# l646773422/h264-lab

Measured on AMD Instinct MI355X. Metric: 1080p macroblocks/sec, higher is better.
Workload: dtype u8

## Files before the change

h264-lab_amd/csrc/enc_mb.h:

```cpp
#ifndef H264E_ENC_MB_H
#define H264E_ENC_MB_H

#include <stddef.h>
#include "enc_kernels.h"

struct GCtx { mv32 mv_left[4], mv_tl[4], mv_top[8]; };
#define GSCR_OFF(t) ((t) == 0 ? 0 : (t) == 1 ? 1024 : (t) == 2 ? 1536 : 2048)
#define GSCR_BYTES 2304

struct MbBuf
{
    alignas(16) uint8_t inp[256];
    alignas(16) uint8_t inp_c[128];
    alignas(16) uint8_t pred[256];
    alignas(4) uint8_t pix_top[36];
    alignas(4) uint8_t ptop[96];
    mv32 mv_top[8];
    uint8_t nnz_top[8];
    int8_t i4_top[4];
    uint32_t df_nz_top;
    int top_type, top_qp;
    mv32 mv[16], mvd[16];
    int type, cost, used_cand;
    mv32 mv_skip_pred;
// ... 248 lines not shown
        v = mvadd(mv, mvmk(DX(pri) + DX(sec), DY(pri) + DY(sec)));
        if (in_rect(v, range))
        {
            cost = grp_sad_ref(R, px + (mvx(v) >> 2), py + (mvy(v) >> 2), b, w, h) + mv_cost(m, v, mv_pred);
            if (cost < min_sad)
            {
                mv = v;
                min_sad = cost;
                continue;
            }
        }
        break;
    }
    STAMP(L, 25);
#undef SEL4
#undef DX
#undef DY

#ifdef H264E_ABLATE
    if (H264E_ABLATE == 3) { grp_interp_luma(R, px, py, mv, w, h, dst); return min_sad; }
#endif
    if (!(m.speed < 9 && in_rect(mv, mv_qlimit(m))))
    {
        grp_interp_luma(R, px, py, mv, w, h, dst);
        return min_sad;
    }
    {
        mv32 pq = mvmk(0, -1), sq = mvmk(-1, 0);
        uint32_t ms1 = c1, ms2 = c3;
        if (c3 >= c2) { pq = mvmk(0, 1); ms2 = c2; }
        if (c1 >= c0) { sq = mvmk(1, 0); ms1 = c0; }
        if (ms2 > ms1) { mv32 sw = sq; sq = pq; pq = sw; }
        const mv32 vdg = mvadd(pq, sq);
        const mv32 v02 = mvadd(mv, mvadd(pq, pq)), v01 = mvadd(mv, pq), v20 = mvadd(mv, mvadd(sq, sq)), v10 = mvadd(mv, sq);
        const mv32 v11 = mvadd(mv, vdg), v22 = mvadd(mv, mvadd(vdg, vdg)), v12 = mvadd(mv, mvadd(pq, vdg));
        int s8[8];
        const int fx0 = px + (mvx(mv) >> 2), fy0 = py + (mvy(mv) >> 2), plane = w*h;
        const bool inside = rv_inside(R, fx0 - 5, fy0 - 3, fx0 + w + 4, fy0 + h + 3);
        if (!inside) rv_wait_rect_g(R, fy0 - 3, fx0 + w + 4, fy0 + h + 3);
        const int hp_ox = mvx(vdg) < 0 ? 1 : 0, hp_oy = mvy(vdg) < 0 ? 1 : 0, hp_pq_vertical = mvx(pq) == 0;
#define AVG4(x, y) (((x) | (y)) - ((((x) ^ (y)) >> 1) & 0x7f7f7f7fu))
        grp_sum8([&](int i, int *sv) {
            uint32_t t0 = 0, t1 = 0, t2 = 0, t3 = 0, t4 = 0, t5 = 0, t6 = 0;
            const int c4 = i & (g - 1), r0 = (i >> (g >> 1))*npass;
            const auto probe = [&](int r, uint32_t q00, uint32_t q02, uint32_t q20, uint32_t q22) {
                const int o = w*r + 4*c4;
                const uint32_t in4 = lds32(b + 16*r + 4*c4);
                const uint32_t q01 = AVG4(q00, q02), q10 = AVG4(q00, q20), q11 = AVG4(q02, q20), q12 = AVG4(q22, q02);
                lds32_store(scr + o, q00); lds32_store(scr + plane + o, q02); lds32_store(scr + 2*plane + o, q20); lds32_store(scr + 3*plane + o, q22);
                t0 = sad4_u8(q02, in4, t0); t1 = sad4_u8(q01, in4, t1); t2 = sad4_u8(q20, in4, t2);
                t3 = sad4_u8(q10, in4, t3); t4 = sad4_u8(q11, in4, t4); t5 = sad4_u8(q22, in4, t5);
                t6 = sad4_u8(q12, in4, t6);
            };
            if (inside)
            {
                halfpel3_rows(rv_ptr(R, fx0 + 4*c4 - hp_ox, fy0 + r0 - hp_oy), hp_ox, hp_oy, npass, [&](int k, const hp4_t &hp) {
                    probe(r0 + k, hp.x, hp_pq_vertical ? hp.z : hp.y, hp_pq_vertical ? hp.y : hp.z, hp.w);
                });
            } else
            {
                for (int k = 0; k < npass; k++)
                {
                    const int r = r0 + k;
#define IP(vv) interp_luma4(R, false, px + (mvx(vv) >> 2) + 4*c4, py + (mvy(vv) >> 2) + r, mvx(vv) & 3, mvy(vv) & 3)
                    const uint32_t q00 = IP(mv), q02 = IP(v02), q20 = IP(v20), q22 = IP(v22);
#undef IP
                    probe(r, q00, q02, q20, q22);
                }
            }
            sv[0] = (int)t0; sv[1] = (int)t1; sv[2] = (int)t2; sv[3] = (int)t3; sv[4] = (int)t4; sv[5] = (int)t5; sv[6] = (int)t6;
        }, s8);
        wave_sync();
        int best = -1, c8[8];
        mv32 vbest = mv;
        {
            const int pax = hp_pq_vertical, p_step = pax ? mvy(pq) : mvx(pq), s_step = pax ? mvx(sq) : mvy(sq);
            const int p_mv = pax ? mvy(mv) : mvx(mv), s_mv = pax ? mvx(mv) : mvy(mv), p_pr = pax ? mvy(mv_pred) : mvx(mv_pred), s_pr = pax ? mvx(mv_pred) : mvy(mv_pred);
            int P[4], S[4];
            grp_eval4([&](int k) -> int { return se_len((int16_t)(p_mv + k*p_step) - p_pr); }, P);
            grp_eval4([&](int k) -> int { return se_len((int16_t)(s_mv + k*s_step) - s_pr); }, S);
            c8[0] = MUL_LAMBDA(P[2] + S[0], m.lambda_mv); c8[1] = MUL_LAMBDA(P[1] + S[0], m.lambda_mv); c8[2] = MUL_LAMBDA(P[0] + S[2], m.lambda_mv);
            c8[3] = MUL_LAMBDA(P[0] + S[1], m.lambda_mv); c8[4] = MUL_LAMBDA(P[1] + S[1], m.lambda_mv); c8[5] = MUL_LAMBDA(P[2] + S[2], m.lambda_mv);
            c8[6] = MUL_LAMBDA(P[2] + S[1], m.lambda_mv);
        }
#define TRY(j, vv) { const int cst = s8[j] + c8[j]; if (cst < min_sad) { min_sad = cst; vbest = (vv); best = j; } }
        TRY(0, v02) TRY(1, v01) TRY(2, v20) TRY(3, v10) TRY(4, v11) TRY(5, v22) TRY(6, v12)
#undef TRY
        const int pa = best < 0 ? 0 : best == 0 ? 1 : best == 1 ? 0 : best == 2 ? 2 : best == 3 ? 0 : best == 4 ? 1 : best == 5 ? 3 : 3;
        const int pb = best == 1 ? 1 : best == 3 ? 2 : best == 4 ? 2 : best == 6 ? 1 : pa;
        GRP_FOR(i)
        {
            for (int k = 0; k < npass; k++)
            {
                const int d = i + 16*k, r = d >> (g >> 1), c4 = d & (g - 1), o = w*r + 4*c4;
                const uint32_t x = lds32(scr + pa*plane + o), y = lds32(scr + pb*plane + o);
                lds32_store(dst + 16*r + 4*c4, AVG4(x, y));
            }
        }
#undef AVG4
        wave_sync();
        mv = vbest;
    }
    STAMP(L, 26);
    return min_sad;
}

DEV void search_type(RowLds &L, const MbBuf &B, const MbCtx &m, int t, mv32 mv_best, int sad_best0, const rect_t &lim, int skip_cost)
{
    GCtx &X = L.gctx[t];
    int imv = 0, part_sad = MUL_LAMBDA(t == 0 ? 1 : t == 3 ? 12 : 4, m.lambda_q4);
    const int w = (t & 2) ? 8 : 16, h = (t & 1) ? 8 : 16;
    int px = 0, py = 0;
    uint8_t *test = L.gtest[t], *scr = L.gscr + GSCR_OFF(t);
    for (;;)
    {
        rect_t range;
        mv32 mvabs = mb_abs(m, mv_best);
        int sad_best = sad_best0;
        const mv32 mvp = mvp_get_arr(X.mv_left, X.mv_tl, X.mv_top, m.avail, px >> 2, py >> 2, w >> 2, h >> 2);
        if (!t) set_range(mvabs, range, lim, m.y*64 + py*4);
        else
        {
            mvabs = mvround(mb_abs(m, mvp));
            set_range(mvabs, range, lim, m.y*64 + py*4);
            sad_best = grp_sad_ref(m.rv, px + (mvx(mvabs) >> 2), py + (mvy(mvabs) >> 2), B.inp + 16*py + px, w, h)
                     + mv_cost(m, mvabs, mb_abs(m, mvp));
        }
        STAMP(L, 24);
        part_sad += diamond_g(L, B, m, px, py, mvabs, range, mb_abs(m, mvp), sad_best, w, h, test + 16*py + px, scr);
        const mv32 mv = mvsub(mvabs, mvmk(m.x*64, m.y*64));
        L.part_mvd[t][imv] = mvsub(mv, mvp);
        L.part_mv[t][imv++] = mv;
        mvp_put_arr(X.mv_left, X.mv_tl, X.mv_top, px >> 2, py >> 2, w >> 2, h >> 2, mv);
        wave_sync();
        STAMP(L, 27);
        if (t == 0) L.early_bound = imax(part_sad, skip_cost);
        px = (px + w) & 15;
        if (!px)
        {
            py = (py + h) & 15;
            if (!py) break;
        }
    }
    L.gcost[t] = part_sad;
    L.gnum[t] = imv;
}

DEV void partition_hints(const int sad[4], int mode[4])
{
    int sum = sad[0] + sad[1] + sad[2] + sad[3];
    int slope = iabs((sad[0] - sad[2]) + (sad[1] - sad[3])) - iabs((sad[0] - sad[1]) + (sad[2] - sad[3]));
    int skew = iabs(sad[3] - sad[0]) - iabs(sad[2] - sad[1]);
    if (slope > (sum >> 4)) mode[1] = 1;
    if (slope < -(sum >> 4)) mode[2] = 1;
    if (iabs(skew) > (sum >> 4) && iabs(slope) <= (sum >> 4)) mode[3] = 1;
}

DEV void predict_chroma_inter(const MbBuf &B, const MbCtx &m, uint8_t *pred_c)
{
    int w = (m.type & 2) ? 4 : 8, h = (m.type & 1) ? 4 : 8, part = 0, x = 0, y = 0;
    if (m.type == -1) w = h = 8;
    for (;; part++)
    {
        wave_interp_chroma(m.rv, m.ref[1], m.ref[2], x, y, mb_abs(m, B.mv[part]), w, h, pred_c + 16*y + x);
        x = (x + w) & 7;
        if (!x)
        {
            y = (y + h) & 7;
            if (!y) break;
        }
    }
}

DEV int skip_chroma_ok(const MbBuf &B, const MbCtx &m, const uint8_t *pred_c)
{
    const int thr = m.skip_thr;
    for (int c = 0; c < 2; c++)
    {
// ... 114 lines not shown
        if (kmin != 0x7fffffff && (kmin >> 4) < sad_best + cand_cost_best)
        {
            mv_best = (mv32)cand.get(kmin & 15);
            cand_cost_best = mv_cost(m, mv_best, mv_pred16);
            sad_best = (kmin >> 4) - cand_cost_best;
        }
    }
    sad_best += mv_cost(m, mv_best, mv_pred16);
    {
        int u = MUL_LAMBDA(1, m.lambda_q4) + sad_best;
        if (sad_skip != 0x7FFFFFFF) u = imax(u, sad_skip + mv_cost(m, mv_skip, mv_pred16));
        sig.bound(u);
    }
    STAMP(L, 4);

#ifdef H264E_ABLATE
    if (H264E_ABLATE == 1) prefer[3] = 0;
    if (H264E_ABLATE == 4) prefer[1] = prefer[2] = prefer[3] = 0;
#endif
    const int types = 1 | (prefer[1] ? 2 : 0) | (prefer[2] ? 4 : 0) | (prefer[3] ? 8 : 0);
#ifdef H264E_TYPES_PROBE
    PCOUNT(L, 20 + (types == 1 ? 0 : (types & 8) ? 2 : 1));
#endif
    WAVE_FOR(l)
    {
        const int i = l & 15;
        mv32 *c = &L.gctx[l >> 4].mv_left[0];
        c[i] = i < 4 ? L.mv_left[i] : i < 8 ? L.mv_tl[i - 4] : i < 13 ? B.mv_top[i - 8] : 0;
    }
    wave_sync();
    const bool helped = sig.helper() && (types & 8);
    if (helped) sig.t3_request(mv_best, sad_best, lim);
    const int types_here = helped ? types & 7 : types;
    GRP_EACH(t)
    {
        if ((types_here >> t) & 1) search_type(L, B, m, t, mv_best, sad_best, lim, sad_skip != 0x7FFFFFFF ? sad_skip + mv_cost(m, mv_skip, mv_pred16) : 0);
    }
    wave_sync();
    if (helped && !sig.t3_wait()) { m.type = 0; m.cost = 0xffffff; B.mv[0] = 0; B.mvd[0] = 0; return; }
    STAMP(L, 5);
    m.cost = 0xffffff;
    int best_n = 0;
    for (int t = 0; t < 4; t++)
        if ((types >> t) & 1)
        {
            const int c = uni(L.gcost[t]);
            if (c < m.cost) { m.cost = c; m.type = t; best_n = uni(L.gnum[t]); }
        }
    wave_copy_wh(B.pred, L.gtest[m.type], 16, 16);
    for (int i = 0; i < best_n; i++) { B.mv[i] = L.part_mv[m.type][i]; B.mvd[i] = L.part_mvd[m.type][i]; }
    wave_sync();

    if (m.cost > sad_skip)
    {
        m.type = 0;
        m.cost = sad_skip + mv_cost(m, mv_skip, mv_pred16);
        B.mv[0] = mv_skip;
        B.mvd[0] = mvsub(mv_skip, mv_pred16);
        wave_copy_wh(B.pred, L.skip_pred, 16, 16);
    }
}


DEV int intra16_cost(RowLds &L, const MbBuf &B, MbCtx &m)
{
    const uint8_t *p = B.inp;
    const int v = m.avail & 3;
    int mode, sad4[4];
    int dx = iabs(p[0] - p[15]) + iabs(p[15*16] - p[15*16 + 15]) + iabs(p[8*16] - p[8*16 + 15]);
// ... 322 lines not shown
```

h264-lab_amd/csrc/enc_row.h:

```cpp
#ifndef H264E_ENC_ROW_H
#define H264E_ENC_ROW_H

#include "enc_mb.h"

#define GEOM_WIDE 0
#define GEOM_NARROW 1
#define GEOM_INTRA 2

struct ChainG
{
    GLOBAL_AS h264e_mbbottom_t *bottom;
    GLOBAL_AS h264e_mbpend_t *pend;
    GLOBAL_AS int *progress;
    GLOBAL_AS uint32_t *rowbits;
    GLOBAL_AS h264e_rowmeta_t *rowmeta;
    GLOBAL_AS h264e_mbrec_t *mbrec;
    GLOBAL_AS uint8_t *arena;
    uint32_t arena_cap;
    GLOBAL_AS uint8_t *nal_arena;
    uint32_t nal_cap;
    GLOBAL_AS uint32_t *cursor;
    GLOBAL_AS h264e_frameout_t *fout;
    GLOBAL_AS int *far_reads;
    unsigned long long *prof;
};
DEV ChainG chain_view(const h264e_chain_dev_t &C)
{
    ChainG g;
    g.bottom = (GLOBAL_AS h264e_mbbottom_t *)C.bottom; g.pend = (GLOBAL_AS h264e_mbpend_t *)C.pend; g.progress = (GLOBAL_AS int *)C.progress;
    g.rowbits = (GLOBAL_AS uint32_t *)C.rowbits; g.rowmeta = (GLOBAL_AS h264e_rowmeta_t *)C.rowmeta;
    g.mbrec = (GLOBAL_AS h264e_mbrec_t *)C.mbrec; g.arena = (GLOBAL_AS uint8_t *)C.arena; g.arena_cap = C.arena_cap; g.nal_arena = (GLOBAL_AS uint8_t *)C.nal_arena; g.nal_cap = C.nal_cap;
    g.cursor = (GLOBAL_AS uint32_t *)C.cursor; g.fout = (GLOBAL_AS h264e_frameout_t *)C.fout; g.far_reads = (GLOBAL_AS int *)C.far_reads; g.prof = C.prof;
    return g;
}

DEV void row_begin(RowLds &L, const h264e_geom_t &G, const ChainG &C, const h264e_frame_task_t &T, int row)
{
    WAVE_FOR(l)
    {
        if (l < 4) { L.mv_left[l] = 0; L.mv_tl[l] = 0; L.i4_left[l] = -1; L.pix_tl[l] = 0; }
        if (l < 8) L.nnz_left[l] = NNZ_NA;
        if (l < 32) L.pix_left[l] = 0;
        if (l < 25) L.df_mv[l] = 0;
        L.strip_y[l] = 0;
        L.strip_c[l >> 5][l & 31] = 0;
    }
    L.df_nzflag = 0;
    L.left_type = 0;
    L.left_qp = T.qp;
    L.bw.acc = 0; L.bw.nacc = 0; L.bw.pos = 0; L.bw.overflow = 0;
    L.bw.cap = (uint32_t)G.row_words;
    L.bw.buf = C.rowbits + (size_t)row*G.row_words;
    L.skip_run = 0; L.lead_skips = 0; L.coded_any = 0; L.far_reads[0] = L.far_reads[1] = L.far_reads[2] = 0; L.far_fail[0] = L.far_fail[1] = L.far_fail[2] = 0;
    L.f_noskip = L.f_bound = L.f_inter = L.f_decided = L.f_wdone = L.f_stop = 0; L.early_bound = 0; L.f_t3req = L.f_t3done = L.f_front = 0;
    WAVE_FOR(l) { if (l <= H264E_MAX_SLICES) L.slice_row[l] = l <= T.nslices ? T.slice_row[l] : (int16_t)0x7fff; }
    WAVE_FOR(l)
    {
        for (int k = l; k < 84; k += 64) L.qdat[k/42][k%42] = T.qdat[k/42][k%42];
    }
    cavlc_tab_load(L.cavlc);
    df_tab_load(L.dftab);
    L.qconst[0] = k_lambda_mv_q4[T.qp]; L.qconst[1] = k_lambda_q4[T.qp]; L.qconst[2] = k_skip_thr_inter[T.qp];
    L.qconst[3] = k_skip_thr_i4x4[T.qp]; L.qconst[4] = k_lambda_i4_q4[T.qp]; L.qconst[5] = k_lambda_i16_q4[T.qp];
    L.win_x = -2;
#ifdef H264E_STAMPS
// ... 734 lines not shown
```

h264-lab_amd/csrc/h264e_kernels.hip:

```cpp
#include <stdio.h>
#include <stdlib.h>
#include <string.h>
#include "enc_row.h"
#include "enc_selftest.h"
#include "enc_denoise.h"
#include "enc_ingest.h"
#include "enc_egress.h"
#include "enc_scale.h"
#include "enc_scale_rgb.h"
#include "enc_hbd.h"
#include "enc_scenecut.h"
#include "enc_ssim.h"
#include "../../include/h264e_hip.h"

#include <hip/hip_runtime.h>





#ifndef H264E_POLL_SLEEP
#define H264E_POLL_SLEEP 16
#endif
DEV int poll_progress(const GLOBAL_AS int *flag, int need, int &seen, unsigned spin_limit)
// ... 46 lines not shown
};
struct InterFromSearchWave
{
    RowLds *L;
    int need;
    bool back_wave;
    DEVM bool before_decide() const { return !back_wave || need < 2 || lds_wait(&L->f_wdone, need - 1, &L->f_stop) == 0; }
    DEVM bool ready() const { return uni(flag_get(&L->f_inter)) >= need; }
    DEVM bool wait_ready() const { return lds_wait(&L->f_inter, need, &L->f_stop) == 0; }
    DEVM int early_bound() const { return uni(flag_get(&L->f_bound)) >= need ? uni(L->early_bound) : 0x7fffffff; }
    DEVM bool wait_either(const int *f) const
    {
        for (unsigned spins = 0;; spins++)
        {
            if (uni(flag_get(&L->f_inter)) >= need || uni(flag_get(f)) >= need) return true;
            if (uni(flag_get(&L->f_stop))) return false;
            if (spins > LDS_SPIN_LIMIT) { flag_set(&L->f_stop, -1); return false; }
            __builtin_amdgcn_s_sleep(H264E_LDS_SLEEP);
        }
    }
    DEVM bool wait_noskip_or_ready() const { return wait_either(&L->f_noskip); }
    DEVM bool wait_bound_or_ready() const { return wait_either(&L->f_bound); }
};

#ifndef H264E_WPE2
#define H264E_WPE2 3
#endif
#ifndef H264E_WPE1
#define H264E_WPE1 2
#endif
#ifndef H264E_WPEI
#define H264E_WPEI 4
#endif
template <int GEOM, int WAVES, int OCC>
__global__ void __launch_bounds__(64*WAVES, OCC) h264e_mb_kernel(h264e_geom_t G, const h264e_frame_task_t *tasks, const uint32_t *order)
{
    __shared__ __attribute__((aligned(16))) unsigned char L_bytes[GEOM == GEOM_INTRA ? ROWLDS_INTRA_BYTES : sizeof(RowLds)];
    RowLds &L = *reinterpret_cast<RowLds *>(L_bytes);
    const int wv = WAVES >= 2 ? __builtin_amdgcn_readfirstlane((int)(threadIdx.x >> 6)) : 0;
#ifdef H264E_LDS_PAD
    __shared__ volatile char lds_pad[H264E_LDS_PAD];
    if (G.nmbx < 0) lds_pad[LANE] = 1;
#endif
    const uint32_t jr = order[blockIdx.x];
    if (jr == H264E_ORDER_PAD) return;
    const int job = (int)(jr >> 16), row = (int)(jr & 0xffffu);
    const h264e_frame_task_t &T = tasks[job];
    if (!T.active) return;
    const ChainG C = chain_view(*T.chain_desc);
    GLOBAL_AS int *errflag = (GLOBAL_AS int *)uniptr(T.errflag);

    if (row == G.nmby)
    {
        if (wv) return;
#ifdef H264E_STAMPS
        unsigned long long fz_t = wall_clock64();
#define FZ_STAMP(id) do { const unsigned long long n_ = wall_clock64(); if (LANE == 0 && C.prof) atomicAdd(C.prof + (id), n_ - fz_t); fz_t = n_; } while (0)
#else
#define FZ_STAMP(id) do { } while (0)
#endif
        int st = 0, seen = 0;
        GLOBAL_AS h264e_hostdone_t *hd = (GLOBAL_AS h264e_hostdone_t *)T.host_done;
        GLOBAL_AS h264e_walkrec_t *wout = (GLOBAL_AS h264e_walkrec_t *)T.walk_out;
        int wstatus = 0, first_bad = -1, have_prev = !(T.walk_on_device && T.walk_prev), published = 0;
        mv32 ws[2] = { T.exact_state[0], T.exact_state[1] };
        const GLOBAL_AS h264e_walkrec_t *wp = (const GLOBAL_AS h264e_walkrec_t *)T.walk_prev;
        const GLOBAL_AS h264e_mbrec_t *rec = C.mbrec + (size_t)T.frame_slot*G.nmb;
        JobWalk W;
        W.begin(ws);
        const bool state_fixed = T.nslices > 1;
        const auto take_prev = [&]() {
            __builtin_amdgcn_fence(__ATOMIC_ACQUIRE, "agent");
            asm volatile("s_waitcnt vmcnt(0)" ::: "memory");
            __builtin_amdgcn_wave_barrier();
            if (uni(wp->status) != H264E_WALK_OK) wstatus = H264E_WALK_VOID;
            else if (!state_fixed) { ws[0] = (mv32)uni(wp->state_out[0]); ws[1] = (mv32)uni(wp->state_out[1]); W.begin(ws); }
            have_prev = 1;
// ... 136 lines not shown
    if (row < T.first_row) return;
    if (job == 0 && row == G.test_stall_row) return;
    if (wv == 0) row_begin(L, G, C, T, row);
    if (WAVES >= 2) __syncthreads();
    const RowTask RT = rowtask_load(T);
    int row0 = 0, row1 = G.nmby;
    for (int k = 0; k < T.nslices; k++)
        if (row >= T.slice_row[k] && row < T.slice_row[k + 1]) { row0 = T.slice_row[k]; row1 = T.slice_row[k + 1]; }
    row0 = uni(row0); row1 = uni(row1);
    GLOBAL_AS int *my_progress = C.progress + row;
    GLOBAL_AS unsigned long long *mb_counter = (GLOBAL_AS unsigned long long *)uniptr(T.mb_counter);
    const auto count_mbs = [&](int n) { if (mb_counter && n > 0 && LANE == 0) __hip_atomic_fetch_add(mb_counter, (unsigned long long)n, __ATOMIC_RELAXED, __HIP_MEMORY_SCOPE_AGENT); };

    if (WAVES == 1 || wv == 0)
    {
        const GLOBAL_AS int *abort_word = (const GLOBAL_AS int *)uniptr(T.abort_word);
        const int launch_id = uni(T.launch_id);
        int seen = 0, seen_dep = 0;
        constexpr bool NARROW = GEOM == GEOM_NARROW;
        constexpr int DEP_ROWS = NARROW ? H264E_NARROW_DEP_ROWS : H264E_DEP_ROWS, DEP_COLS = NARROW ? H264E_NARROW_DEP_COLS : H264E_DEP_COLS;
        unsigned long long deps = 0;
        int ndeps = 0;
        if (T.dep_progress)
        {
            const int lo = imax(row - 2, 0), hi = imin(row + DEP_ROWS, G.nmby - 1);
            deps = (unsigned long long)hi; ndeps = 1;
            for (int k = T.nslices - 1; k >= 1; k--)
            {
                const int last = T.slice_row[k] - 1;
                if (last >= lo && last < hi) { deps |= (unsigned long long)last << (10*ndeps); ndeps++; }
            }
            ndeps = uni(ndeps);
        }
        for (int x = 0; x < G.nmbx; x++)
        {
            const int need = row > row0 ? imin(x + 2, G.nmbx) : 0;
            const int need_dep = RT.dep_progress ? imin(x + DEP_COLS, G.nmbx) : 0;
            int st = 0;
            const int abort_v = abort_word ? __hip_atomic_load(abort_word, __ATOMIC_RELAXED, __HIP_MEMORY_SCOPE_AGENT) : launch_id - 1;
            const GLOBAL_AS int *above = C.progress + (WAVES >= 2 ? G.nmby : 0) + (row - 1);
            const int early = seen < need ? __hip_atomic_load(above, __ATOMIC_RELAXED, __HIP_MEMORY_SCOPE_AGENT) : seen;
            if (seen_dep < need_dep)
            {
                int lowest = 0x7fffffff;
                for (int k = 0; k < ndeps && !st; k++)
                {
                    int sk = 0;
                    st = poll_progress((const GLOBAL_AS int *)RT.dep_progress + (int)((deps >> (10*k)) & 1023), need_dep, sk, G.spin_limit);
                    lowest = imin(lowest, sk);
                }
                seen_dep = lowest;
                if (!st) consumer_acquire();
            }
            STAMP(L, 13);
            if (WAVES >= 2 && !st && x >= 2) st = lds_wait(&L.f_wdone, x - 1, &L.f_stop);
            STAMP(L, 23);
            if (!st) row_prefetch<GEOM>(L, G, RT, row, x);
            STAMP(L, 0);
            if (uni(abort_v) == launch_id) st = -2;
            if (!st && seen < need)
            {
                seen = uni(early);
                if (seen < 0) st = seen;
                else if (seen < need) st = poll_progress(above, need, seen, G.spin_limit);
                if (!st) consumer_acquire();
            }
            STAMP(L, 13);
            if (!st) load_top<WAVES >= 2 ? LOAD_TOP_MV : LOAD_TOP_ALL>(L, L.mb[x & 1], G, C.bottom + (size_t)(row - 1)*G.nmbx, C.pend + (size_t)(row - 1)*G.nmbx, x, row > row0);
            STAMP(L, 0);
            if (WAVES >= 2 && !st && x >= 1) st = lds_wait(&L.f_decided, x, &L.f_stop);
            STAMP(L, 6);
            if (st)
            {
                if (WAVES >= 2) { flag_set(&L.f_stop, st); return; }
                if (LANE == 0)
                {
                    if (st == -1) *errflag = 1;
                    __hip_atomic_store(my_progress, st, __ATOMIC_RELAXED, __HIP_MEMORY_SCOPE_AGENT);
                }
                count_mbs(x);
                return;
            }
            if (WAVES == 1) row_step<GEOM>(L, G, C, RT, row, x, row0, row1);
            else mb_search<GEOM>(L, L.mb[x & 1], G, RT, row, x, row0, SearchSignals{ &L, x + 1, WAVES >= 3 });
            if (WAVES >= 3 && uni(flag_get(&L.f_stop))) return;
            {
                const int ff = uni(L.far_fail[0]) | (WAVES == 1 ? uni(L.far_fail[1]) : 0);
                if (ff)
                {
                    if (WAVES >= 2) { flag_set(&L.f_stop, ff < -2 ? -2 : ff); return; }
                    if (LANE == 0)
                    {
                        if (ff == -1) *errflag = 1;
                        __hip_atomic_store(my_progress, ff < -2 ? -2 : ff, __ATOMIC_RELAXED, __HIP_MEMORY_SCOPE_AGENT);
                    }
                    count_mbs(x);
                    return;
                }
            }
            if (WAVES >= 2) { flag_set(&L.f_inter, x + 1); STAMP(L, 14); continue; }
            asm volatile("s_waitcnt vmcnt(0)" ::: "memory");
// ... 459 lines not shown
```

h264-lab_amd/csrc/h264e_pool.h:

```cpp
#ifndef H264E_POOL_H
#define H264E_POOL_H
#include "enc_denoise.h"
#include "enc_ingest.h"
#include "enc_egress.h"
#include "enc_scale.h"
#include "enc_scale_rgb.h"
#include "enc_hbd.h"
#include "enc_scenecut.h"
#include "enc_ssim.h"

static const h264e_color_t k_color_rows[4] = {
    { { 66, 129, 25 }, { -38, -74, 112 }, { 112, -94, -18 }, 16 },
    { { 77, 150, 29 }, { -43, -84, 127 }, { 127, -107, -20 }, 0 },
    { { 47, 157, 16 }, { -26, -86, 112 }, { 112, -102, -10 }, 16 },
    { { 54, 183, 19 }, { -29, -98, 127 }, { 127, -116, -11 }, 0 } };

static const h264e_icolor_t k_icolor_rows[4] = {
    { 298, 16, 409, -100, -208, 516 },
    { 256, 0, 359, -88, -183, 454 },
    { 298, 16, 459, -55, -136, 541 },
    { 256, 0, 403, -48, -120, 475 } };

static thread_local char g_err[256];
#define FAIL(...) do { snprintf(g_err, sizeof(g_err), __VA_ARGS__); return -1; } while (0)
// ... 1294 lines not shown
        (void)hipMemset(p->errflag, 0, sizeof(int));
        FAIL("macroblock kernel gave up waiting for the row above (bounded spin expired)");
    }
    device_release(p);
    p->pending = 0;
    return 0;
}

extern "C" void h264e_hip_release(h264e_hip_pool_t *p)
{
    if (!p) return;
    (void)hipSetDevice(p->device);
    if (p->stream) (void)hipStreamSynchronize(p->stream);
    device_release(p);
}


extern "C" int h264e_hip_group_create(h264e_hip_group_t **out, int device)
{
    if (!out) FAIL("group_create: null argument");
    h264e_hip_group_t *g = (h264e_hip_group_t *)calloc(1, sizeof(*g));
    if (!g) FAIL("out of host memory");
    g->device = device;
    pthread_mutex_init(&g->mu, 0); pthread_cond_init(&g->cv, 0);
    if (hipSetDevice(device) != hipSuccess || hipStreamCreate(&g->stream) != hipSuccess) { free(g); FAIL("group_create: no stream on device %d", device); }
    (void)hipEventCreate(&g->ev_done);
    for (int k = 0; k < 2; k++) { (void)hipEventCreate(&g->ev_t0[k]); (void)hipEventCreate(&g->ev_t1[k]); }
    *out = g;
    return 0;
}

#define H264E_RESIDENT_WG_V2 1536
#define H264E_RESIDENT_WG_V3 512
static int pick_variant(const launch_shape_t &s, int jobs, int nmby)
{
    if (s.forced) return s.forced;
    if (s.all_intra) return 0;
    if (jobs*nmby >= H264E_RESIDENT_WG_V2 && s.parallel && !s.tree) return 4;
    if (jobs*(nmby + 1) <= H264E_RESIDENT_WG_V3) return 3;
    return 2;
}

static hipError_t launch_mb(const h264e_geom_t &G, int narrow, int variant, int jobs, size_t nblocks, const h264e_frame_task_t *tasks, const uint32_t *order,
                            hipEvent_t before, hipEvent_t after, hipStream_t stream)
{
    hipError_t e = before ? hipEventRecord(before, stream) : hipSuccess;
    if (e != hipSuccess) return e;
    bk_launch_mb(G, narrow, variant, jobs, (unsigned)nblocks, tasks, order, stream);
    e = after ? hipEventRecord(after, stream) : hipSuccess;
    const hipError_t le = hipGetLastError();
    return le != hipSuccess ? le : e;
}

static int group_fail(h264e_hip_group_t *g, const char *fmt, ...)
{
    va_list ap;
    va_start(ap, fmt);
    vsnprintf(g->err, sizeof(g->err), fmt, ap);
    va_end(ap);
    return -1;
}

static int group_grow(h264e_hip_group_t *g, void **buf, size_t *cap, size_t need, size_t slack, size_t elem)
{
    if (need <= *cap) return 0;
    if (*buf) (void)hipFree(*buf);
    *cap = need + slack;
    if (hipMalloc(buf, elem**cap) == hipSuccess) return 0;
    *buf = 0; *cap = 0;
    return group_fail(g, "group launch: device allocation failed");
}
// ... 556 lines not shown
```

h264-lab_amd/csrc/wave.h:

```cpp
#ifndef H264E_WAVE_H
#define H264E_WAVE_H

#include <stdint.h>
#include <string.h>

#ifdef H264E_EMU
extern "C" void emu_check_global(const void *p, size_t n, const char *file, int line);
#define EMU_GLOBAL(p, n) emu_check_global((const void *)(p), (n), __FILE__, __LINE__)
#define GLOBAL_AS
#define LDS_AS
#define NOINLINE_DEV static __attribute__((noinline))
#define DEV static inline
#define DEVM inline
#define DCONST static const
#ifdef H264E_EMU_REVERSE
#define WAVE_FOR(l) for (int l = 63; l >= 0; --l)
#else
#define WAVE_FOR(l) for (int l = 0; l < 64; ++l)
#endif
struct u32x4 { uint32_t x, y, z, w; };
DEV void wave_sync() {}
DEV int wave_lane() { return 0; }
DEV int uni(int v) { return v; }
template <class F> DEV int wave_sum(F f)
// ... 11 lines not shown
        f(l, v);
        for (int k = 0; k < 4; ++k) out[k] += v[k];
    }
}
template <class F> DEV void wave_sum8(F f, int out[8])
{
    for (int k = 0; k < 8; ++k) out[k] = 0;
    for (int l = 0; l < 64; ++l)
    {
        int v[8] = { 0, 0, 0, 0, 0, 0, 0, 0 };
        f(l, v);
        for (int k = 0; k < 8; ++k) out[k] += v[k];
    }
}
template <class F> DEV uint64_t wave_ballot(F f)
{
    uint64_t m = 0;
    for (int l = 0; l < 64; ++l) if (f(l)) m |= 1ull << l;
    return m;
}
DEV uint32_t sad4_u8(uint32_t a, uint32_t b, uint32_t acc)
{
    for (int k = 0; k < 4; ++k)
    {
        int d = (int)((a >> (8*k)) & 255) - (int)((b >> (8*k)) & 255);
        acc += (uint32_t)(d < 0 ? -d : d);
    }
    return acc;
}
DEV int clz32(uint32_t v) { return __builtin_clz(v); }
DEV uint32_t bswap32(uint32_t v) { return __builtin_bswap32(v); }

#define GRP_EACH(g) for (int g = 0; g < 4; ++g)
#ifdef H264E_EMU_REVERSE
#define GRP_FOR(i) for (int i = 15; i >= 0; --i)
#else
#define GRP_FOR(i) for (int i = 0; i < 16; ++i)
#endif
template <class F> DEV int grp_sum(F f)
{
    int s = 0;
    for (int i = 0; i < 16; ++i) s += f(i);
    return s;
}
template <class F> DEV void grp_sum4(F f, int out[4])
{
    out[0] = out[1] = out[2] = out[3] = 0;
    for (int i = 0; i < 16; ++i)
    {
        int v[4] = { 0, 0, 0, 0 };
        f(i, v);
        for (int k = 0; k < 4; ++k) out[k] += v[k];
    }
}
template <class F> DEV void grp_sum8(F f, int out[8])
{
    for (int k = 0; k < 8; ++k) out[k] = 0;
    for (int i = 0; i < 16; ++i)
    {
        int v[8] = { 0, 0, 0, 0, 0, 0, 0, 0 };
        f(i, v);
        for (int k = 0; k < 8; ++k) out[k] += v[k];
    }
}
template <class F> DEV void grp_eval4(F f, int out[4]) { for (int d = 0; d < 4; ++d) out[d] = f(d); }
template <class F> DEV void grp_eval8(F f, int out[8]) { for (int d = 0; d < 8; ++d) out[d] = f(d); }
DEV void grp_count(int *p) { *p += 1; }

struct V16 { int v[16]; };
#define V16_BINOP(op) DEV V16 operator op(const V16 &a, const V16 &b) { V16 r; for (int i = 0; i < 16; i++) r.v[i] = a.v[i] op b.v[i]; return r; }
V16_BINOP(+) V16_BINOP(-) V16_BINOP(*) V16_BINOP(&) V16_BINOP(|)
#undef V16_BINOP
DEV V16 operator>>(const V16 &a, int s) { V16 r; for (int i = 0; i < 16; i++) r.v[i] = a.v[i] >> s; return r; }
DEV V16 v16_splat(int s) { V16 r; for (int i = 0; i < 16; i++) r.v[i] = s; return r; }
template <class F> DEV V16 v16_make(F f) { V16 r; for (int i = 0; i < 16; i++) r.v[i] = f(i, 0); return r; }
template <class F> DEV V16 v16_map(const V16 &a, F f) { V16 r; for (int i = 0; i < 16; i++) r.v[i] = f(i, a.v[i]); return r; }
template <class F> DEV V16 v16_map2(const V16 &a, const V16 &b, F f) { V16 r; for (int i = 0; i < 16; i++) r.v[i] = f(i, a.v[i], b.v[i]); return r; }
template <class F> DEV V16 v16_map3(const V16 &a, const V16 &b, const V16 &c, F f) { V16 r; for (int i = 0; i < 16; i++) r.v[i] = f(i, a.v[i], b.v[i], c.v[i]); return r; }
template <class F> DEV void v16_each(const V16 &a, F f) { for (int i = 0; i < 16; i++) f(i, 0, a.v[i]); }
DEV int v16_any(const V16 &a) { for (int i = 0; i < 16; i++) if (a.v[i]) return 1; return 0; }
DEV V16 v16_tile_any(const V16 &a) { V16 r; const int n = v16_any(a); for (int i = 0; i < 16; i++) r.v[i] = n; return r; }
DEV unsigned v16_tiles_nonzero(const V16 &a) { return (unsigned)v16_any(a); }
struct V16C { };
DEV V16C v16c_make() { return V16C(); }
template <class F> DEV V16 v16_make(const V16C &, F f) { return v16_make(f); }
template <class F> DEV V16 v16_map(const V16C &, const V16 &a, F f) { return v16_map(a, f); }
template <class F> DEV V16 v16_map2(const V16C &, const V16 &a, const V16 &b, F f) { return v16_map2(a, b, f); }
template <class F> DEV V16 v16_map3(const V16C &, const V16 &a, const V16 &b, const V16 &c, F f) { return v16_map3(a, b, c, f); }
template <class F> DEV void v16_each(const V16C &, const V16 &a, F f) { v16_each(a, f); }
DEV V16 v16_tile_any(const V16C &, const V16 &a) { return v16_tile_any(a); }
template <class V> DEV V v16_fwd4x4_c(const V16C &, const V &d) { return v16_fwd4x4(d); }
template <class V> DEV V v16_inv4x4_c(const V16C &, const V &c) { return v16_inv4x4(c); }
template <int P0, int P1, int P2, int P3> DEV V16 v16_quadperm(const V16 &a)
{
    const int p[4] = { P0, P1, P2, P3 };
    V16 r;
    for (int i = 0; i < 16; i++) r.v[i] = a.v[(i & ~3) | p[i & 3]];
    return r;
}
DEV V16 v16_xpose(const V16 &a) { V16 r; for (int i = 0; i < 16; i++) r.v[i] = a.v[(i & 3)*4 + (i >> 2)]; return r; }
// ... 64 lines not shown
    v += __builtin_amdgcn_update_dpp(0, v, 0x141, 0xf, 0xf, true);
    v += __builtin_amdgcn_update_dpp(0, v, 0x140, 0xf, 0xf, true);
    return __builtin_amdgcn_readlane(v, 0) + __builtin_amdgcn_readlane(v, 16) +
           __builtin_amdgcn_readlane(v, 32) + __builtin_amdgcn_readlane(v, 48);
}
template <class F> DEV int wave_sum(F f) { return wave_reduce_add(f(LANE)); }
template <class F> DEV void wave_sum4(F f, int out[4])
{
    int v[4] = { 0, 0, 0, 0 };
    f(LANE, v);
    int a = v[0] | (v[1] << 16), b = v[2] | (v[3] << 16);
    a = wave_reduce_add(a);
    b = wave_reduce_add(b);
    out[0] = a & 0xffff; out[1] = (int)((unsigned)a >> 16);
    out[2] = b & 0xffff; out[3] = (int)((unsigned)b >> 16);
}
template <class F> DEV void wave_sum8(F f, int out[8])
{
    int v[8] = { 0, 0, 0, 0, 0, 0, 0, 0 };
    f(LANE, v);
#pragma unroll
    for (int k = 0; k < 4; k++)
    {
        int a = wave_reduce_add(v[2*k] | (v[2*k + 1] << 16));
        out[2*k] = a & 0xffff; out[2*k + 1] = (int)((unsigned)a >> 16);
    }
}
template <class F> DEV uint64_t wave_ballot(F f) { return __ballot(f(LANE)); }
DEV uint32_t sad4_u8(uint32_t a, uint32_t b, uint32_t acc) { return __builtin_amdgcn_sad_u8(a, b, acc); }
DEV int clz32(uint32_t v) { return __clz((int)v); }
DEV uint32_t bswap32(uint32_t v) { return __builtin_bswap32(v); }

#define GRP_EACH(g) for (int g = LANE >> 4, _e1 = 1; _e1; _e1 = 0)
#define GRP_FOR(i) for (int i = LANE & 15, _g1 = 1; _g1; _g1 = 0)
DEV int row_reduce_add(int v)
{
    v += __builtin_amdgcn_update_dpp(0, v, 0xB1, 0xf, 0xf, true);
    v += __builtin_amdgcn_update_dpp(0, v, 0x4E, 0xf, 0xf, true);
    v += __builtin_amdgcn_update_dpp(0, v, 0x141, 0xf, 0xf, true);
    v += __builtin_amdgcn_update_dpp(0, v, 0x140, 0xf, 0xf, true);
    return v;
}
template <class F> DEV int grp_sum(F f) { return row_reduce_add(f(LANE & 15)); }
template <class F> DEV void grp_sum4(F f, int out[4])
{
    int v[4] = { 0, 0, 0, 0 };
    f(LANE & 15, v);
    const int a = row_reduce_add(v[0] | (v[1] << 16)), b = row_reduce_add(v[2] | (v[3] << 16));
    out[0] = a & 0xffff; out[1] = (int)((unsigned)a >> 16);
    out[2] = b & 0xffff; out[3] = (int)((unsigned)b >> 16);
}
template <class F> DEV void grp_sum8(F f, int out[8])
{
    int v[8] = { 0, 0, 0, 0, 0, 0, 0, 0 };
    f(LANE & 15, v);
#pragma unroll
    for (int k = 0; k < 4; k++)
    {
        const int a = row_reduce_add(v[2*k] | (v[2*k + 1] << 16));
        out[2*k] = a & 0xffff; out[2*k + 1] = (int)((unsigned)a >> 16);
    }
}
template <class F> DEV void grp_eval4(F f, int out[4])
{
    const int c = f(LANE & 3);
    out[0] = __builtin_amdgcn_update_dpp(0, c, 0x00, 0xf, 0xf, true); out[1] = __builtin_amdgcn_update_dpp(0, c, 0x55, 0xf, 0xf, true);
    out[2] = __builtin_amdgcn_update_dpp(0, c, 0xAA, 0xf, 0xf, true); out[3] = __builtin_amdgcn_update_dpp(0, c, 0xFF, 0xf, 0xf, true);
}
template <class F> DEV void grp_eval8(F f, int out[8])
{
    const int c0 = f(LANE & 3), c1 = f(4 + (LANE & 3));
    out[0] = __builtin_amdgcn_update_dpp(0, c0, 0x00, 0xf, 0xf, true); out[1] = __builtin_amdgcn_update_dpp(0, c0, 0x55, 0xf, 0xf, true);
    out[2] = __builtin_amdgcn_update_dpp(0, c0, 0xAA, 0xf, 0xf, true); out[3] = __builtin_amdgcn_update_dpp(0, c0, 0xFF, 0xf, 0xf, true);
    out[4] = __builtin_amdgcn_update_dpp(0, c1, 0x00, 0xf, 0xf, true); out[5] = __builtin_amdgcn_update_dpp(0, c1, 0x55, 0xf, 0xf, true);
    out[6] = __builtin_amdgcn_update_dpp(0, c1, 0xAA, 0xf, 0xf, true); out[7] = __builtin_amdgcn_update_dpp(0, c1, 0xFF, 0xf, 0xf, true);
}
DEV void grp_count(int *p) { if ((LANE & 15) == 0) __hip_atomic_fetch_add(p, 1, __ATOMIC_RELAXED, __HIP_MEMORY_SCOPE_WORKGROUP); }

struct V16 { int v; };
#define V16_BINOP(op) DEV V16 operator op(const V16 &a, const V16 &b) { V16 r; r.v = a.v op b.v; return r; }
V16_BINOP(+) V16_BINOP(-) V16_BINOP(*) V16_BINOP(&) V16_BINOP(|)
#undef V16_BINOP
DEV V16 operator>>(const V16 &a, int s) { V16 r; r.v = a.v >> s; return r; }
DEV V16 v16_splat(int s) { V16 r; r.v = s; return r; }
template <class F> DEV V16 v16_make(F f) { V16 r; r.v = f(LANE & 15, LANE >> 4); return r; }
template <class F> DEV V16 v16_map(const V16 &a, F f) { V16 r; r.v = f(LANE & 15, a.v); return r; }
template <class F> DEV V16 v16_map2(const V16 &a, const V16 &b, F f) { V16 r; r.v = f(LANE & 15, a.v, b.v); return r; }
template <class F> DEV V16 v16_map3(const V16 &a, const V16 &b, const V16 &c, F f) { V16 r; r.v = f(LANE & 15, a.v, b.v, c.v); return r; }
template <class F> DEV void v16_each(const V16 &a, F f) { f(LANE & 15, LANE >> 4, a.v); }
DEV int v16_any(const V16 &a) { return __ballot(a.v != 0) != 0; }
DEV V16 v16_tile_any(const V16 &a)
{
    const unsigned long long m = __ballot(a.v != 0);
    const int t = LANE >> 4;
    const unsigned w = (t & 2) ? (unsigned)(m >> 32) : (unsigned)m;
    V16 r;
    r.v = ((w >> (16*(t & 1))) & 0xffffu) != 0;
    return r;
}
DEV unsigned v16_tiles_nonzero(const V16 &a)
{
    const unsigned long long m = __ballot(a.v != 0);
    const unsigned lo = (unsigned)m, hi = (unsigned)(m >> 32);
    return ((lo & 0xffffu) ? 1u : 0u) | ((lo >> 16) ? 2u : 0u) | ((hi & 0xffffu) ? 4u : 0u) | ((hi >> 16) ? 8u : 0u);
}
template <int P0, int P1, int P2, int P3> DEV V16 v16_quadperm(const V16 &a)
{
    V16 r;
    r.v = __builtin_amdgcn_update_dpp(0, a.v, P0 | (P1 << 2) | (P2 << 4) | (P3 << 6), 0xf, 0xf, true);
    return r;
// ... 205 lines not shown
```

Measured before the change: 13.90 million.

## Cut VGPR pressure in motion search and widen V4 variant selection

Several unrelated changes are combined. Subpel refinement candidates are now rebuilt from a nibble-packed table instead of seven live vectors. search_type gets its per-group type from the lane id, accumulates partition cost in LDS with an atomic add, and writes MV slots by computed index. Kernel arguments and pointers are marked wave-uniform so they can sit in scalar registers. The pool also picks the V4 variant for short frames even when not parallel, and a static_assert guards the LDS budget. Together these aim to lower vector-register use and raise occupancy, at the cost of LDS atomics and a behaviour change in which variant is chosen.

```diff
diff --git a/h264-lab_amd/csrc/enc_mb.h b/h264-lab_amd/csrc/enc_mb.h
--- a/h264-lab_amd/csrc/enc_mb.h
+++ b/h264-lab_amd/csrc/enc_mb.h
@@ -304,8 +304,6 @@
         if (c1 >= c0) { sq = mvmk(1, 0); ms1 = c0; }
         if (ms2 > ms1) { mv32 sw = sq; sq = pq; pq = sw; }
         const mv32 vdg = mvadd(pq, sq);
-        const mv32 v02 = mvadd(mv, mvadd(pq, pq)), v01 = mvadd(mv, pq), v20 = mvadd(mv, mvadd(sq, sq)), v10 = mvadd(mv, sq);
-        const mv32 v11 = mvadd(mv, vdg), v22 = mvadd(mv, mvadd(vdg, vdg)), v12 = mvadd(mv, mvadd(pq, vdg));
         int s8[8];
         const int fx0 = px + (mvx(mv) >> 2), fy0 = py + (mvy(mv) >> 2), plane = w*h;
         const bool inside = rv_inside(R, fx0 - 5, fy0 - 3, fx0 + w + 4, fy0 + h + 3);
@@ -335,6 +333,7 @@
                 {
                     const int r = r0 + k;
 #define IP(vv) interp_luma4(R, false, px + (mvx(vv) >> 2) + 4*c4, py + (mvy(vv) >> 2) + r, mvx(vv) & 3, mvy(vv) & 3)
+                    const mv32 v02 = mvadd(mv, mvadd(pq, pq)), v20 = mvadd(mv, mvadd(sq, sq)), v22 = mvadd(mv, mvadd(vdg, vdg));
                     const uint32_t q00 = IP(mv), q02 = IP(v02), q20 = IP(v20), q22 = IP(v22);
 #undef IP
                     probe(r, q00, q02, q20, q22);
@@ -344,7 +343,6 @@
         }, s8);
         wave_sync();
         int best = -1, c8[8];
-        mv32 vbest = mv;
         {
             const int pax = hp_pq_vertical, p_step = pax ? mvy(pq) : mvx(pq), s_step = pax ? mvx(sq) : mvy(sq);
             const int p_mv = pax ? mvy(mv) : mvx(mv), s_mv = pax ? mvx(mv) : mvy(mv), p_pr = pax ? mvy(mv_pred) : mvx(mv_pred), s_pr = pax ? mvx(mv_pred) : mvy(mv_pred);
@@ -355,9 +353,14 @@
             c8[3] = MUL_LAMBDA(P[0] + S[1], m.lambda_mv); c8[4] = MUL_LAMBDA(P[1] + S[1], m.lambda_mv); c8[5] = MUL_LAMBDA(P[2] + S[2], m.lambda_mv);
             c8[6] = MUL_LAMBDA(P[2] + S[1], m.lambda_mv);
         }
-#define TRY(j, vv) { const int cst = s8[j] + c8[j]; if (cst < min_sad) { min_sad = cst; vbest = (vv); best = j; } }
-        TRY(0, v02) TRY(1, v01) TRY(2, v20) TRY(3, v10) TRY(4, v11) TRY(5, v22) TRY(6, v12)
+#define TRY(j) { const int cst = s8[j] + c8[j]; if (cst < min_sad) { min_sad = cst; best = j; } }
+        TRY(0) TRY(1) TRY(2) TRY(3) TRY(4) TRY(5) TRY(6)
 #undef TRY
+        if (best >= 0)
+        {
+            const int a = (0x2210012 >> (4*best)) & 15, c = (0x1211200 >> (4*best)) & 15;
+            mv = mvmk(mvx(mv) + a*mvx(pq) + c*mvx(sq), mvy(mv) + a*mvy(pq) + c*mvy(sq));
+        }
         const int pa = best < 0 ? 0 : best == 0 ? 1 : best == 1 ? 0 : best == 2 ? 2 : best == 3 ? 0 : best == 4 ? 1 : best == 5 ? 3 : 3;
         const int pb = best == 1 ? 1 : best == 3 ? 2 : best == 4 ? 2 : best == 6 ? 1 : pa;
         GRP_FOR(i)
@@ -371,7 +374,6 @@
         }
 #undef AVG4
         wave_sync();
-        mv = vbest;
     }
     STAMP(L, 26);
     return min_sad;
@@ -379,19 +381,23 @@
 
 DEV void search_type(RowLds &L, const MbBuf &B, const MbCtx &m, int t, mv32 mv_best, int sad_best0, const rect_t &lim, int skip_cost)
 {
-    GCtx &X = L.gctx[t];
-    int imv = 0, part_sad = MUL_LAMBDA(t == 0 ? 1 : t == 3 ? 12 : 4, m.lambda_q4);
-    const int w = (t & 2) ? 8 : 16, h = (t & 1) ? 8 : 16;
+    L.gcost[t] = MUL_LAMBDA(t == 0 ? 1 : t == 3 ? 12 : 4, m.lambda_q4);
+    L.gnum[t] = t == 0 ? 1 : t == 3 ? 4 : 2;
     int px = 0, py = 0;
-    uint8_t *test = L.gtest[t], *scr = L.gscr + GSCR_OFF(t);
     for (;;)
     {
+        const int tg = GRP_ID(t), w = (tg & 2) ? 8 : 16, h = (tg & 1) ? 8 : 16;
+        GCtx &X = L.gctx[tg];
         rect_t range;
-        mv32 mvabs = mb_abs(m, mv_best);
-        int sad_best = sad_best0;
         const mv32 mvp = mvp_get_arr(X.mv_left, X.mv_tl, X.mv_top, m.avail, px >> 2, py >> 2, w >> 2, h >> 2);
-        if (!t) set_range(mvabs, range, lim, m.y*64 + py*4);
-        else
+        mv32 mvabs;
+        int sad_best;
+        if (!tg)
+        {
+            mvabs = mb_abs(m, mv_best);
+            sad_best = sad_best0;
+            set_range(mvabs, range, lim, m.y*64 + py*4);
+        } else
         {
             mvabs = mvround(mb_abs(m, mvp));
             set_range(mvabs, range, lim, m.y*64 + py*4);
@@ -399,23 +405,27 @@
                      + mv_cost(m, mvabs, mb_abs(m, mvp));
         }
         STAMP(L, 24);
-        part_sad += diamond_g(L, B, m, px, py, mvabs, range, mb_abs(m, mvp), sad_best, w, h, test + 16*py + px, scr);
-        const mv32 mv = mvsub(mvabs, mvmk(m.x*64, m.y*64));
-        L.part_mvd[t][imv] = mvsub(mv, mvp);
-        L.part_mv[t][imv++] = mv;
-        mvp_put_arr(X.mv_left, X.mv_tl, X.mv_top, px >> 2, py >> 2, w >> 2, h >> 2, mv);
-        wave_sync();
-        STAMP(L, 27);
-        if (t == 0) L.early_bound = imax(part_sad, skip_cost);
-        px = (px + w) & 15;
-        if (!px)
-        {
-            py = (py + h) & 15;
-            if (!py) break;
-        }
-    }
-    L.gcost[t] = part_sad;
-    L.gnum[t] = imv;
+        const int cost = diamond_g(L, B, m, px, py, mvabs, range, mb_abs(m, mvp), sad_best, w, h, L.gtest[tg] + 16*py + px, L.gscr + GSCR_OFF(tg));
+        {
+            const int tq = GRP_ID(t), wq = (tq & 2) ? 8 : 16, hq = (tq & 1) ? 8 : 16;
+            GCtx &Y = L.gctx[tq];
+            const int imv = (px >> 3) + ((py >> 3) << (wq == 8 ? 1 : 0));
+            const mv32 mv = mvsub(mvabs, mvmk(m.x*64, m.y*64));
+            L.part_mvd[tq][imv] = mvsub(mv, mvp);
+            L.part_mv[tq][imv] = mv;
+            grp_add(&L.gcost[tq], cost);
+            mvp_put_arr(Y.mv_left, Y.mv_tl, Y.mv_top, px >> 2, py >> 2, wq >> 2, hq >> 2, mv);
+            wave_sync();
+            STAMP(L, 27);
+            if (tq == 0) L.early_bound = imax(MUL_LAMBDA(1, m.lambda_q4) + cost, skip_cost);
+            px = (px + wq) & 15;
+            if (!px)
+            {
+                py = (py + hq) & 15;
+                if (!py) break;
+            }
+        }
+    }
 }
 
 DEV void partition_hints(const int sad[4], int mode[4])
@@ -596,9 +606,13 @@
     const bool helped = sig.helper() && (types & 8);
     if (helped) sig.t3_request(mv_best, sad_best, lim);
     const int types_here = helped ? types & 7 : types;
-    GRP_EACH(t)
-    {
-        if ((types_here >> t) & 1) search_type(L, B, m, t, mv_best, sad_best, lim, sad_skip != 0x7FFFFFFF ? sad_skip + mv_cost(m, mv_skip, mv_pred16) : 0);
+    {
+        const mv32 mv_start = (mv32)uni(mv_best);
+        const int sad_start = uni(sad_best), skip_cost = uni(sad_skip != 0x7FFFFFFF ? sad_skip + mv_cost(m, mv_skip, mv_pred16) : 0);
+        GRP_EACH(t)
+        {
+            if ((types_here >> t) & 1) search_type(L, B, m, t, mv_start, sad_start, lim, skip_cost);
+        }
     }
     wave_sync();
     if (helped && !sig.t3_wait()) { m.type = 0; m.cost = 0xffffff; B.mv[0] = 0; B.mvd[0] = 0; return; }
diff --git a/h264-lab_amd/csrc/enc_row.h b/h264-lab_amd/csrc/enc_row.h
--- a/h264-lab_amd/csrc/enc_row.h
+++ b/h264-lab_amd/csrc/enc_row.h
@@ -27,10 +27,11 @@
 DEV ChainG chain_view(const h264e_chain_dev_t &C)
 {
     ChainG g;
-    g.bottom = (GLOBAL_AS h264e_mbbottom_t *)C.bottom; g.pend = (GLOBAL_AS h264e_mbpend_t *)C.pend; g.progress = (GLOBAL_AS int *)C.progress;
-    g.rowbits = (GLOBAL_AS uint32_t *)C.rowbits; g.rowmeta = (GLOBAL_AS h264e_rowmeta_t *)C.rowmeta;
-    g.mbrec = (GLOBAL_AS h264e_mbrec_t *)C.mbrec; g.arena = (GLOBAL_AS uint8_t *)C.arena; g.arena_cap = C.arena_cap; g.nal_arena = (GLOBAL_AS uint8_t *)C.nal_arena; g.nal_cap = C.nal_cap;
-    g.cursor = (GLOBAL_AS uint32_t *)C.cursor; g.fout = (GLOBAL_AS h264e_frameout_t *)C.fout; g.far_reads = (GLOBAL_AS int *)C.far_reads; g.prof = C.prof;
+    g.bottom = uniptr((GLOBAL_AS h264e_mbbottom_t *)C.bottom); g.pend = uniptr((GLOBAL_AS h264e_mbpend_t *)C.pend); g.progress = uniptr((GLOBAL_AS int *)C.progress);
+    g.rowbits = uniptr((GLOBAL_AS uint32_t *)C.rowbits); g.rowmeta = uniptr((GLOBAL_AS h264e_rowmeta_t *)C.rowmeta);
+    g.mbrec = uniptr((GLOBAL_AS h264e_mbrec_t *)C.mbrec); g.arena = uniptr((GLOBAL_AS uint8_t *)C.arena); g.arena_cap = (uint32_t)uni((int)C.arena_cap);
+    g.nal_arena = uniptr((GLOBAL_AS uint8_t *)C.nal_arena); g.nal_cap = (uint32_t)uni((int)C.nal_cap);
+    g.cursor = uniptr((GLOBAL_AS uint32_t *)C.cursor); g.fout = uniptr((GLOBAL_AS h264e_frameout_t *)C.fout); g.far_reads = uniptr((GLOBAL_AS int *)C.far_reads); g.prof = uniptr(C.prof);
     return g;
 }
 
diff --git a/h264-lab_amd/csrc/h264e_kernels.hip b/h264-lab_amd/csrc/h264e_kernels.hip
--- a/h264-lab_amd/csrc/h264e_kernels.hip
+++ b/h264-lab_amd/csrc/h264e_kernels.hip
@@ -102,6 +102,9 @@
 #ifndef H264E_WPEI
 #define H264E_WPEI 4
 #endif
+#if !defined(H264E_STAMPS) && !defined(H264E_LDS_PAD)
+static_assert(sizeof(RowLds) + 16 <= 20480, "RowLds (+ 16 B of alignment) must fit 160 KB / 8: the 4-per-SIMD two-wave variants keep 8 workgroups per CU");
+#endif
 template <int GEOM, int WAVES, int OCC>
 __global__ void __launch_bounds__(64*WAVES, OCC) h264e_mb_kernel(h264e_geom_t G, const h264e_frame_task_t *tasks, const uint32_t *order)
 {
@@ -112,7 +115,7 @@
     __shared__ volatile char lds_pad[H264E_LDS_PAD];
     if (G.nmbx < 0) lds_pad[LANE] = 1;
 #endif
-    const uint32_t jr = order[blockIdx.x];
+    const uint32_t jr = (uint32_t)uni((int)order[blockIdx.x]);
     if (jr == H264E_ORDER_PAD) return;
     const int job = (int)(jr >> 16), row = (int)(jr & 0xffffu);
     const h264e_frame_task_t &T = tasks[job];
@@ -315,6 +318,7 @@
             }
             ndeps = uni(ndeps);
         }
+        const int above_mb = uni((row - 1)*G.nmbx);
         for (int x = 0; x < G.nmbx; x++)
         {
             const int need = row > row0 ? imin(x + 2, G.nmbx) : 0;
@@ -349,7 +353,7 @@
                 if (!st) consumer_acquire();
             }
             STAMP(L, 13);
-            if (!st) load_top<WAVES >= 2 ? LOAD_TOP_MV : LOAD_TOP_ALL>(L, L.mb[x & 1], G, C.bottom + (size_t)(row - 1)*G.nmbx, C.pend + (size_t)(row - 1)*G.nmbx, x, row > row0);
+            if (!st) load_top<WAVES >= 2 ? LOAD_TOP_MV : LOAD_TOP_ALL>(L, L.mb[x & 1], G, C.bottom + above_mb, C.pend + above_mb, x, row > row0);
             STAMP(L, 0);
             if (WAVES >= 2 && !st && x >= 1) st = lds_wait(&L.f_decided, x, &L.f_stop);
             STAMP(L, 6);
diff --git a/h264-lab_amd/csrc/h264e_pool.h b/h264-lab_amd/csrc/h264e_pool.h
--- a/h264-lab_amd/csrc/h264e_pool.h
+++ b/h264-lab_amd/csrc/h264e_pool.h
@@ -1350,11 +1350,12 @@
 
 #define H264E_RESIDENT_WG_V2 1536
 #define H264E_RESIDENT_WG_V3 512
+#define H264E_V4_SHORT_ROWS 45
 static int pick_variant(const launch_shape_t &s, int jobs, int nmby)
 {
     if (s.forced) return s.forced;
     if (s.all_intra) return 0;
-    if (jobs*nmby >= H264E_RESIDENT_WG_V2 && s.parallel && !s.tree) return 4;
+    if (jobs*nmby >= H264E_RESIDENT_WG_V2 && (s.parallel || nmby <= H264E_V4_SHORT_ROWS) && !s.tree) return 4;
     if (jobs*(nmby + 1) <= H264E_RESIDENT_WG_V3) return 3;
     return 2;
 }
diff --git a/h264-lab_amd/csrc/wave.h b/h264-lab_amd/csrc/wave.h
--- a/h264-lab_amd/csrc/wave.h
+++ b/h264-lab_amd/csrc/wave.h
@@ -67,6 +67,7 @@
 DEV uint32_t bswap32(uint32_t v) { return __builtin_bswap32(v); }
 
 #define GRP_EACH(g) for (int g = 0; g < 4; ++g)
+#define GRP_ID(g) (g)
 #ifdef H264E_EMU_REVERSE
 #define GRP_FOR(i) for (int i = 15; i >= 0; --i)
 #else
@@ -101,6 +102,7 @@
 template <class F> DEV void grp_eval4(F f, int out[4]) { for (int d = 0; d < 4; ++d) out[d] = f(d); }
 template <class F> DEV void grp_eval8(F f, int out[8]) { for (int d = 0; d < 8; ++d) out[d] = f(d); }
 DEV void grp_count(int *p) { *p += 1; }
+DEV void grp_add(int *p, int v) { *p += v; }
 
 struct V16 { int v[16]; };
 #define V16_BINOP(op) DEV V16 operator op(const V16 &a, const V16 &b) { V16 r; for (int i = 0; i < 16; i++) r.v[i] = a.v[i] op b.v[i]; return r; }
@@ -231,6 +233,7 @@
 DEV uint32_t bswap32(uint32_t v) { return __builtin_bswap32(v); }
 
 #define GRP_EACH(g) for (int g = LANE >> 4, _e1 = 1; _e1; _e1 = 0)
+#define GRP_ID(g) ((void)(g), LANE >> 4)
 #define GRP_FOR(i) for (int i = LANE & 15, _g1 = 1; _g1; _g1 = 0)
 DEV int row_reduce_add(int v)
 {
@@ -275,6 +278,7 @@
     out[6] = __builtin_amdgcn_update_dpp(0, c1, 0xAA, 0xf, 0xf, true); out[7] = __builtin_amdgcn_update_dpp(0, c1, 0xFF, 0xf, 0xf, true);
 }
 DEV void grp_count(int *p) { if ((LANE & 15) == 0) __hip_atomic_fetch_add(p, 1, __ATOMIC_RELAXED, __HIP_MEMORY_SCOPE_WORKGROUP); }
+DEV void grp_add(int *p, int v) { if ((LANE & 15) == 0) __hip_atomic_fetch_add(p, v, __ATOMIC_RELAXED, __HIP_MEMORY_SCOPE_WORKGROUP); }
 
 struct V16 { int v; };
 #define V16_BINOP(op) DEV V16 operator op(const V16 &a, const V16 &b) { V16 r; r.v = a.v op b.v; return r; }
```

Result: no change. 13.93 million (median of 6 runs) (+0.2%).
